# tlangin/MDQTPlasmaSims

Hardware: AMD Instinct MI355X
Metric: particle-steps/sec (MD+QT) at N=3.5k and N=1M; 1/2/4/8-GPU scaling (higher is better)
Workload: dtype f64

## Files before the change

mdqtplasmasims_amd/csrc/mdqt_engine.cpp:

```cpp
#include <errno.h>
#include <math.h>
#include <stdarg.h>
#include <stdio.h>
#include <stdlib.h>
#include <string.h>
#include <sys/stat.h>

#include <string>
#include <algorithm>
#include <memory>
#include <thread>
#include <vector>

#include <rccl/rccl.h>

#include "../../include/mdqt.h"
#include "mdqt_internal.hpp"
#include "mdqt_writer.hpp"
#include "mdqt_init_sample.hpp"

using namespace mdqt;

namespace {

// ... 124 lines not shown
    int fused_opt = 0;
    int last_fused = 0;
    int last_qt_kernel = 0;
    int last_qt_nseg = 0;
    int* dSpinErr = nullptr;
    unsigned long long* force_arrive = nullptr;
    hipStream_t sub_stream = nullptr;
    unsigned long long sub_target = 0;
    std::vector<int> spinUp;
    int nSpinUp = 0;
    int* dSpinUp = nullptr;
    double* dTkde = nullptr;
    int pumpBin0 = -2000;
    std::vector<double> vaHold;
    bool rs_pending = false;
    const double** dPeerParts = nullptr;
    int nslots = 0, npairs = 0, capPairs = 0;
    int2* dPairs = nullptr;
    int nsplit = 0;
    int nsplit_wg = 0;
    int split_opt = 1;
    int split_cus = 0;
    unsigned long long* dX48 = nullptr;
    int* dFlags = nullptr;
    bool guard = false;
    double* dU = nullptr;
    ncclComm_t comm = nullptr;
    double* dComm = nullptr;
    std::vector<mdqt_ctx*> local;
    size_t dCommCap = 0;
    double t = 0.;
    uint64_t qidx = 0;
    int c0 = 0;
    unsigned counter = 0;
    double Epot = 0., Epot0 = 0.;
    uint64_t x48 = 0;
    std::vector<double> Vholder;
    char saveDirectory[1024];
    std::unique_ptr<FileWriter> writer;
    FileWriter* shared_writer = nullptr;
    int init_threads = 0;
    bool timing = false;
    unsigned tkinds = 3;
    unsigned tperiod = 1, tcount[2] = {0, 0};
    unsigned toffset = 0;
    std::vector<hipEvent_t> evpool[4];
    int evused[4] = {0, 0, 0, 0};
    struct BdCall { hipEvent_t ag0 = nullptr, ag1 = nullptr; hipEvent_t m[7] = {}; };
    std::vector<BdCall> bdcalls;
    std::vector<hipEvent_t> bdfree;
    hipEvent_t bd_ag[2] = {nullptr, nullptr};
};

static int settle_forces(mdqt_ctx* s);
static int tail_check(mdqt_ctx* s);
static double u64_as_double(unsigned long long u) { double d; memcpy(&d, &u, sizeof d); return d; }

static int tail_reset(mdqt_ctx* s, bool keep_scale = false) {
    if (!keep_scale) s->tail_scale = 1.;
    s->tail_seen = 0;
    s->tail_pending = false;
    if (s->dTailSt) HIPCHK(hipMemsetAsync(s->dTailSt, 0, 16 * sizeof(unsigned long long), s->stream));
    return 0;
}

static int check_range_flag(mdqt_ctx* s) {
    if (s->dSpinErr) {
        int e = 0;
        if (hipMemcpyAsync(&e, s->dSpinErr, sizeof e, hipMemcpyDeviceToHost, s->stream) != hipSuccess ||
            hipStreamSynchronize(s->stream) != hipSuccess)
            return fail("reading the overlap flag failed");
        if (e) return fail("overlapped MD step: a QT launch timed out waiting for its force launch");
    }
    int f = 0;
    if (hipMemcpyAsync(&f, s->dFlags, sizeof f, hipMemcpyDeviceToHost, s->stream) != hipSuccess ||
        hipStreamSynchronize(s->stream) != hipSuccess)
        return fail("reading the position-range flag failed");
    if (f && !s->guard) {
        s->guard = true;
        return fail("positions left [-L/8, 9L/8] during the run (ion displacement > L/8 per half "
                    "substep); pair range checks are now on, but forces since the last sync used "
                    "the in-box minimum image");
    }
    return tail_check(s);
}


extern "C" void mdqt_default_params(mdqt_params* p) {
    memset(p, 0, sizeof(*p));
    p->Ge = 0.1; p->tmax = 30; p->density = 2; p->sig0 = 4.0; p->Te = 19.0; p->fracOfSig = 0;
    p->detuning = -1; p->detuningDP = 1; p->Om = 1; p->OmDP = 1;
    p->N0 = 3500; p->newRun = 1; p->c0 = 0; p->sampleFreq = 40; p->reNormalizewvFns = 0;
    p->qt_enabled = 1; p->rng_mode = 1; p->seed = 12345; p->job = 1;
    p->device = -1; p->world_size = 1; p->rank = 0; p->force_segments = 0; p->qt_model = 0;
    strcpy(p->saveDirectory, "dataLaserCool/");
    p->tpumpreal = 0.0000002; p->tstartV0 = 15;
}

extern "C" void mdqt_default_params_pump(mdqt_params* p, int qt_model) {
    mdqt_default_params(p);
    p->qt_model = qt_model;
    p->tmax = 25; p->Ge = 0.1; p->density = 2; p->N0 = 3500; p->sampleFreq = 40; p->tstartV0 = 15;
    if (qt_model == 2) {
        p->detuning = 0; p->Om = 2; p->tpumpreal = 0.0000001; strcpy(p->saveDirectory, "data/");
    } else if (qt_model == 3) {
        p->detuning = -1; p->Om = 1.3; p->tpumpreal = 0.0000001; strcpy(p->saveDirectory, "data422/");
    } else {
// ... 524 lines not shown
        return fail("the optical-pumping qt_models run on the Philox stream (rng_mode 1)");
    int ndev = 0;
    hipError_t e = hipGetDeviceCount(&ndev);
    if (e != hipSuccess || ndev < 1) return fail("no HIP device available (%s)", hipGetErrorString(e));
    mdqt_ctx* s = new mdqt_ctx();
    s->p = *p;
    s->p.saveDirectory[sizeof(s->p.saveDirectory) - 1] = 0;
    if (p->device >= 0) {
        if (p->device >= ndev) { delete s; return fail("device %d >= device count %d", p->device, ndev); }
        s->dev = p->device;
    } else {
        (void)hipGetDevice(&s->dev);
    }
    if (hipSetDevice(s->dev) != hipSuccess || hipStreamCreateWithFlags(&s->own, hipStreamNonBlocking) != hipSuccess) {
        delete s;
        return fail("cannot create HIP stream on device %d", p->device);
    }
    s->stream = s->own;
    if (hipMalloc(&s->dTab, sizeof(LaneTab)) != hipSuccess || hipMalloc(&s->dFTab, 2 * sizeof(FastTab)) != hipSuccess) {
        mdqt_destroy(s);
        return fail("hipMalloc lane tables");
    }
    {
        const int f[2] = {0, 1};
        if (hipMalloc(&s->dFlags, sizeof f) != hipSuccess ||
            hipMemcpy(s->dFlags, f, sizeof f, hipMemcpyHostToDevice) != hipSuccess) {
            mdqt_destroy(s);
            return fail("hipMalloc flags");
        }
    }
    build_constants(s);
    if (s->p.rng_mode == 0) {
        unsigned long long h[97];
        h[0] = srand48_state(s->p.seed);
        unsigned long long A = 0x5DEECE66Dull, Cc = 0xBull;
        for (int b = 0; b < 48; ++b) {
            h[1 + b] = A; h[49 + b] = Cc;
            Cc = (A * Cc + Cc) & 0xFFFFFFFFFFFFull;
            A = (A * A) & 0xFFFFFFFFFFFFull;
        }
        if (hipMalloc(&s->dX48, sizeof h) != hipSuccess ||
            hipMemcpy(s->dX48, h, sizeof h, hipMemcpyHostToDevice) != hipSuccess) {
            mdqt_destroy(s);
            return fail("drand48 state upload failed");
        }
    }
    if (hipMemcpy(s->dTab, &s->tab, sizeof(LaneTab), hipMemcpyHostToDevice) != hipSuccess ||
        hipMemcpy(s->dFTab, &s->ftab, sizeof(FastTab), hipMemcpyHostToDevice) != hipSuccess ||
        hipMemcpy(s->dFTab + 1, &s->ftabL, sizeof(FastTab), hipMemcpyHostToDevice) != hipSuccess) {
        mdqt_destroy(s);
        return fail("upload of the lane table failed");
    }
    s->t = 0.; s->qidx = 0; s->c0 = p->c0; s->counter = 0;
    s->x48 = srand48_state(p->seed);
    strncpy(s->saveDirectory, s->p.saveDirectory, sizeof(s->saveDirectory) - 1);
    s->saveDirectory[sizeof(s->saveDirectory) - 1] = 0;
    if (resize(s, 0)) { mdqt_destroy(s); return -1; }
    *out = s;
    return 0;
}

extern "C" void mdqt_destroy(mdqt_ctx* s) {
    if (!s) return;
    s->writer.reset();
    (void)hipSetDevice(s->dev);
    if (s->stream) (void)hipStreamSynchronize(s->stream);
    free_device(s);
    if (s->dTab) (void)hipFree(s->dTab);
    if (s->dFTab) (void)hipFree(s->dFTab);
    if (s->dComm) (void)hipFree(s->dComm);
    if (s->dSpinUp) (void)hipFree(s->dSpinUp);
    if (s->dArrive) (void)hipFree(s->dArrive);
    if (s->dSpinErr) (void)hipFree(s->dSpinErr);
    if (s->evQ) (void)hipEventDestroy(s->evQ);
    if (s->evS) (void)hipEventDestroy(s->evS);
    if (s->qs) (void)hipStreamDestroy(s->qs);
    if (s->dTkde) (void)hipFree(s->dTkde);
    if (s->dX48) (void)hipFree(s->dX48);
    if (s->dFlags) (void)hipFree(s->dFlags);
    if (s->comm) (void)ncclCommDestroy(s->comm);
    for (auto& pool : s->evpool)
        for (hipEvent_t ev : pool) (void)hipEventDestroy(ev);
    for (auto& c : s->bdcalls) {
        for (hipEvent_t ev : c.m) if (ev) (void)hipEventDestroy(ev);
        if (c.ag0) (void)hipEventDestroy(c.ag0);
        if (c.ag1) (void)hipEventDestroy(c.ag1);
    }
    for (hipEvent_t ev : s->bdfree) (void)hipEventDestroy(ev);
    for (hipEvent_t ev : s->bd_ag) if (ev) (void)hipEventDestroy(ev);
    if (s->own) (void)hipStreamDestroy(s->own);
    delete s;
}

static double tail_radius(int N, double L, double lDeb, int k, double* bound);
static double tail_radius_sum(const mdqt_ctx* s, double* bound);
static bool tail_measured(const mdqt_ctx* s);
static double skip_radius(const mdqt_ctx* s, double* bound);
static double far_radius(int N, double L, double lDeb, int k, double* bound);
static double far_radius_l(int N, double L, double lDeb, int k, int level, double* bound, bool cutterm = true);
static bool form_measured(const mdqt_ctx* s);
static double tier_radius(const mdqt_ctx* s, int k, int level, double* bound);
static void tier_radii(const mdqt_ctx* s, N3BArgs& a);
static double error_eps(const mdqt_ctx* s, const N3BArgs& a);
extern "C" double mdqt_get_const(const mdqt_ctx* s, const char* n) {
    if (!strcmp(n, "gamToEinsteinFreq")) return s->gamToE;
    if (!strcmp(n, "quantumTimestep")) return s->dtQ;
    if (!strcmp(n, "plasmaToQuantumTimestepRatio")) return s->ratio;
    if (!strcmp(n, "plasVelToQuantVel")) return s->pv2q;
    if (!strcmp(n, "vKick")) return s->vKick;
    if (!strcmp(n, "vKickDP")) return s->vKickDP;
    if (!strcmp(n, "lDeb")) return s->lDeb;
    if (!strcmp(n, "L")) return s->L;
    if (!strcmp(n, "decayRatioD5Halves")) return s->r;
    if (!strcmp(n, "kRat")) return s->kRat;
    if (!strcmp(n, "force_segments")) return s->nseg;
    if (!strcmp(n, "force_scheme")) return s->use_n3b ? 3 : s->use_n3 ? 2 : 1;
    if (!strcmp(n, "force_sort")) return s->use_n3b ? s->sort_mode : 0;
    if (!strcmp(n, "force_ax1")) return s->ax1_mode;
    if (!strcmp(n, "force_reduce_mask")) return s->tmask_mode;
    if (!strcmp(n, "force_tile_split")) return s->split_opt;
    if (!strcmp(n, "force_split_cus")) return s->split_cus;
    if (!strcmp(n, "force_tile_split_pairs")) return s->nsplit;
    if (!strcmp(n, "device_cus")) {
        int ncu = 0;
        return hipDeviceGetAttribute(&ncu, hipDeviceAttributeMultiprocessorCount, s->dev) == hipSuccess ? ncu : -1;
    }
    if (!strcmp(n, "force_balance")) return s->balance_opt;
    if (!strcmp(n, "force_balance_ratio")) return s->balance_ratio;
    if (!strcmp(n, "force_balance_ratio_equal")) return s->balance_ratio_eq;
    if (!strcmp(n, "n3b_block_lo")) return s->use_n3b ? s->n3b.Plo : 0;
    if (!strcmp(n, "n3b_block_hi")) return s->use_n3b ? s->n3b.Phi : 0;
    if (!strcmp(n, "force_skip_radius") || !strcmp(n, "force_tail_bound")) {
        double bound;
        const double r = (s->use_n3b && s->sort_mode == 1) ? skip_radius(s, &bound) : (bound = 0., s->L / 2.);
        if (n[6] == 's') return r;
// ... 82 lines not shown
    if (!strncmp(n, "gs", 2)) return s->gs[atoi(n + 2)];
    return NAN;
}


static int upload(mdqt_ctx* s, const double* R, const double* V, size_t ld, const double* psi,
                  const double* tPart) {
    const int N = s->N, S = s->S, W = s->p.world_size;
    HIPCHK(hipSetDevice(s->dev));
    if (R) {
        std::vector<double> h((size_t)3 * S * W, 0.);
        for (int g = 0; g < N; ++g) {
            const int w = g / S, l = g - w * S;
            for (int c = 0; c < 3; ++c) h[(size_t)w * 3 * S + (size_t)c * S + l] = R[(size_t)c * ld + g];
        }
        HIPCHK(hipMemcpyAsync(s->dR, h.data(), h.size() * sizeof(double), hipMemcpyHostToDevice, s->stream));
        int oor = 0;
        const double plo = -0.125 * s->L, phi = 1.125 * s->L;
        for (size_t k = 0; k < (size_t)3 * N && !oor; ++k) {
            const double x = R[(k / N) * ld + k % N];
            if (!(x >= plo && x <= phi)) oor = 1;
        }
        s->guard = oor != 0;
        const int zero = 0;
        HIPCHK(hipMemcpyAsync(s->dFlags, &zero, sizeof zero, hipMemcpyHostToDevice, s->stream));
        HIPCHK(hipStreamSynchronize(s->stream));
    }
    const int lo = s->lo, n = s->nloc;
    if (V) {
        std::vector<double> h((size_t)3 * S, 0.);
        for (int c = 0; c < 3; ++c)
            for (int i = 0; i < n; ++i) h[(size_t)c * S + i] = V[(size_t)c * ld + lo + i];
        HIPCHK(hipMemcpyAsync(s->dV, h.data(), h.size() * sizeof(double), hipMemcpyHostToDevice, s->stream));
        HIPCHK(hipStreamSynchronize(s->stream));
    }
    if (psi) {
        std::vector<double> h((size_t)24 * S, 0.);
        for (int i = 0; i < n; ++i)
            for (int k = 0; k < 24; ++k) h[(size_t)k * S + i] = psi[(size_t)(lo + i) * 24 + k];
        HIPCHK(hipMemcpyAsync(s->dPsi, h.data(), h.size() * sizeof(double), hipMemcpyHostToDevice, s->stream));
        HIPCHK(hipStreamSynchronize(s->stream));
    }
    if (tPart) {
        std::vector<double> h((size_t)S, 0.);
        for (int i = 0; i < n; ++i) h[i] = tPart[lo + i];
        HIPCHK(hipMemcpyAsync(s->dTp, h.data(), h.size() * sizeof(double), hipMemcpyHostToDevice, s->stream));
        HIPCHK(hipStreamSynchronize(s->stream));
    }
    return 0;
// ... 817 lines not shown
extern "C" int mdqt_step(mdqt_ctx* s) { return s ? run_substeps(s, 1, 1, 0, 0) : fail("NULL context"); }
extern "C" int mdqt_qstep(mdqt_ctx* s) { return s ? run_substeps(s, 1, 0, 1, 1) : fail("NULL context"); }
extern "C" int mdqt_substeps(mdqt_ctx* s, int n) {
    if (!s) return fail("NULL context");
    if (n < 0) return fail("negative substep count");
    return run_substeps(s, n, 1, 1, 1);
}

static bool overlap_applies(const mdqt_ctx* s) {
    return s->overlap_opt && s->p.world_size == 1 && s->local.empty() && s->use_n3 && s->nslots > 1 && s->qt_math == 2 &&
           s->p.qt_enabled && s->p.rng_mode == 1 && s->ratio <= MAXSUB && s->nloc > 0 &&
           (s->substep_mode == 2 || (s->substep_mode == 0 && s->nloc < kLaneKernelMaxIons));
}

static int arrive_setup(mdqt_ctx* s) {
    const int T = (s->N + 63) / 64;
    if (s->dArrive && s->arriveCap >= T) return 0;
    HIPCHK(hipStreamSynchronize(s->stream));
    if (s->qs) HIPCHK(hipStreamSynchronize(s->qs));
    if (s->dArrive) HIPCHK(hipFree(s->dArrive));
    s->dArrive = nullptr;
    HIPCHK(hipMalloc(&s->dArrive, (size_t)T * sizeof(unsigned long long)));
    HIPCHK(hipMemset(s->dArrive, 0, (size_t)T * sizeof(unsigned long long)));
    if (!s->dSpinErr) {
        HIPCHK(hipMalloc(&s->dSpinErr, sizeof(int)));
        HIPCHK(hipMemset(s->dSpinErr, 0, sizeof(int)));
    }
    HIPCHK(hipDeviceSynchronize());
    s->arriveCap = T;
    s->arriveEpoch = 0;
    return 0;
}

static int overlap_setup(mdqt_ctx* s) {
    if (arrive_setup(s)) return -1;
    if (s->qs) return 0;
    HIPCHK(hipStreamCreateWithFlags(&s->qs, hipStreamNonBlocking));
    HIPCHK(hipEventCreateWithFlags(&s->evQ, hipEventDisableTiming | hipEventDisableSystemFence));
    HIPCHK(hipEventCreateWithFlags(&s->evS, hipEventDisableTiming | hipEventDisableSystemFence));
    return 0;
}

static int md_steps_overlapped(mdqt_ctx* s, int n) {
    if (overlap_setup(s)) return -1;
    HIPCHK(hipEventRecord(s->evS, s->stream));
    HIPCHK(hipStreamWaitEvent(s->qs, s->evS, 0));
    for (int k = 0; k < n; ++k) {
        if (k > 0) HIPCHK(hipStreamWaitEvent(s->stream, s->evQ, 0));
        if (k > 0 && k % 64 == 0 && check_range_flag(s)) return -1;
        s->force_arrive = s->dArrive;
        const int rc = mdqt_forces(s);
        s->force_arrive = nullptr;
        if (rc) return -1;
        s->arriveEpoch += (unsigned long long)((s->N + 63) / 64);
        s->c0++;
        s->sub_stream = s->qs;
        s->sub_target = s->arriveEpoch;
        const int rq = run_substeps(s, s->ratio, 1, 1, 1);
        s->sub_stream = nullptr;
        if (rq) return -1;
        HIPCHK(hipEventRecord(s->evQ, s->qs));
    }
    HIPCHK(hipStreamWaitEvent(s->stream, s->evQ, 0));
    return 0;
}

static bool fused_applies(mdqt_ctx* s) {
    if (!(s->fused_opt && !s->overlap_opt && s->p.world_size == 1 && s->local.empty() && s->use_n3 && s->nslots > 1 &&
          s->qt_math == 2 && s->p.qt_enabled && s->p.rng_mode == 1 && s->ratio <= MAXSUB && s->nloc > 0 &&
          s->t > 0 && s->force_variant <= 1 &&
          (s->substep_mode == 2 || (s->substep_mode == 0 && s->nloc < kLaneKernelMaxIons))))
        return false;
// ... 14 lines not shown
    a.nseg = s->nslots;
    a.arrive = s->dArrive;
    a.arrive_target = s->arriveEpoch + T;
    a.spin_err = s->dSpinErr;
    a.arrive_sleep = 2;
    if (a.movmask != (m >= 32 ? 0xFFFFFFFFu : (1u << m) - 1u)) return fail("md_step_fused: t <= 0 in the interval");
    const bool tm = s->timing && (s->tkinds & 2u) && (s->tcount[1]++ % s->tperiod == s->toffset);
    hipEvent_t e0 = nullptr, e1 = nullptr;
    if (tm && take_events(s, 1, &e0, &e1)) return -1;
    HIPCHK(launch_md_step(f, a, s->dFTab, s->force_variant, s->stream, e0, e1));
    s->last_qt_kernel = QTK_MD_STEP;
    s->last_qt_nseg = a.nseg;
    s->arriveEpoch += T;
    s->f_pending = false;
    s->t = t;
    s->qidx += (uint64_t)m;
    return 0;
}

extern "C" int mdqt_md_steps(mdqt_ctx* s, int n) {
    if (!s) return fail("NULL context");
    if (n > 0 && overlap_applies(s)) return md_steps_overlapped(s, n);
    for (int k = 0; k < n; ++k) {
        if (k > 0 && k % 64 == 0 && check_range_flag(s)) return -1;
        if (fused_applies(s)) {
            if (local_reduce(s) || md_step_fused(s)) return -1;
            s->last_fused = 1;
            s->c0++;
            continue;
        }
        s->last_fused = 0;
        if (mdqt_allgather_positions(s)) return -1;
        if (mdqt_forces(s)) return -1;
        s->c0++;
        if (mdqt_substeps(s, s->ratio)) return -1;
    }
    return 0;
}

static int pairs_raw(int mode, int N, double L, double lDeb, const double* R, size_t ld, double* out,
                     int nseg_req, int device, int variant) {
    if (N < 1 || !R || !out || ld < (size_t)N) return fail("pairs_raw: bad arguments");
    if (variant < 0 || variant > 1) return fail("pairs_raw: variant must be 0 (exact) or 1 (fast)");
    int ndev = 0;
    if (hipGetDeviceCount(&ndev) != hipSuccess || ndev < 1) return fail("no HIP device available");
    if (device >= 0) HIPCHK(hipSetDevice(device));
    int lo, hi, S;
// ... 1169 lines not shown
```

mdqtplasmasims_amd/csrc/mdqt_ensemble.hpp:

```cpp
#pragma once

struct mdqt_ensemble {
    std::vector<mdqt_ctx*> jobs;
    int dev = 0;
    hipStream_t stream = nullptr;
    std::unique_ptr<FileWriter> writer;
    N3Args* dForce = nullptr;
    SubstepArgs* dSub = nullptr;
    int sub_blocks = 0;
    std::vector<N3Args> force_held;
    static constexpr int kRing = 8;
    char* ring = nullptr;
    size_t slot_bytes = 0;
    hipEvent_t ring_ev[kRing] = {};
    bool ring_used[kRing] = {};
    unsigned ring_pos = 0;
    int* hFlags = nullptr;
    int qt_waves = 0;
    bool timing = false;
    std::vector<hipEvent_t> evpool[2];
    int evused[2] = {0, 0};
};

namespace {

constexpr int kEnsembleMaxJobs = 1024;

int ens_job_params(const mdqt_params* base, int k, mdqt_params* out) {
    if (!base || !out) return fail("mdqt_ensemble_job_params: NULL argument");
    if (k < 0 || k >= kEnsembleMaxJobs) return fail("mdqt_ensemble_job_params: job index %d outside [0, %d)", k, kEnsembleMaxJobs);
    mdqt_params p = *base;
    p.job = base->job + (uint32_t)k;
    p.seed = base->seed + (uint32_t)k;
    *out = p;
    return 0;
}

int ens_ring_slot(mdqt_ensemble* e, char** slot, int* idx) {
    const int i = (int)(e->ring_pos++ % mdqt_ensemble::kRing);
    if (e->ring_used[i]) HIPCHK(hipEventSynchronize(e->ring_ev[i]));
// ... 108 lines not shown
        for (int k = 0; k < J; ++k) {
            mdqt_ctx* s = e->jobs[k];
            t = substep_args(s, h[k], m, 1, do_qt, 1);
            s->f_pending = false;
            maxn = std::max(maxn, h[k].n);
        }
        if (ens_upload(e, e->dSub, slot, (size_t)J * sizeof(SubstepArgs), idx)) return -1;
        hipEvent_t e0 = nullptr, e1 = nullptr;
        if (e->timing && ens_take_events(e, 1, &e0, &e1)) return -1;
        int inst = 0;
        HIPCHK(launch_substeps_r_ens(e->dSub, h[0], J, maxn, e->jobs[0]->dFTab, e->qt_waves, e->stream, e0, e1, &inst));
        for (int k = 0; k < J; ++k) {
            mdqt_ctx* s = e->jobs[k];
            s->last_qt_kernel = inst;
            s->last_qt_nseg = h[k].nseg;
            s->t = t;
            s->qidx += (uint64_t)m;
        }
        n -= m;
    }
    return 0;
}

int ens_range_flags(mdqt_ensemble* e) {
    const int J = (int)e->jobs.size();
    for (int k = 0; k < J; ++k)
        HIPCHK(hipMemcpyAsync(e->hFlags + k, e->jobs[k]->dFlags, sizeof(int), hipMemcpyDeviceToHost, e->stream));
    HIPCHK(hipStreamSynchronize(e->stream));
    int first = -1;
    for (int k = 0; k < J; ++k)
        if (e->hFlags[k] && !e->jobs[k]->guard) {
            e->jobs[k]->guard = true;
            if (first < 0) first = k;
        }
    if (first >= 0)
        return fail("job index %d: positions left [-L/8, 9L/8] during the run (ion displacement > L/8 per half "
                    "substep); pair range checks are now on, but forces since the last sync used the in-box "
                    "minimum image", first);
    return 0;
}

int ens_md_steps(mdqt_ensemble* e, int n) {
    const int J = (int)e->jobs.size();
    const int ratio = e->jobs[0]->ratio, per_step = (ratio + MAXSUB - 1) / MAXSUB;
    const int do_qt = e->jobs[0]->p.qt_enabled ? 1 : 0;
    bool tiles = true;
    for (const mdqt_ctx* s : e->jobs) tiles = tiles && s->use_n3;
    const int ahead = tiles ? std::min(64, e->sub_blocks / (J * per_step)) : 0;
    if (ahead < 2) {
        for (int k = 0; k < n; ++k) {
            if (k > 0 && k % 64 == 0 && ens_range_flags(e)) return -1;
            if (ens_forces(e)) return -1;
            for (mdqt_ctx* s : e->jobs) s->c0++;
            if (ens_substeps(e, ratio)) return -1;
        }
        return 0;
    }
    for (int k = 0; k < n;) {
        if (k > 0 && k % 64 == 0 && ens_range_flags(e)) return -1;
        const int b = std::min(std::min(n - k, ahead), 64 - k % 64);
        EnsForce f;
        if (ens_force_blocks(e, f)) return -1;
        char* slot = nullptr;
        int idx = 0;
        if (ens_ring_slot(e, &slot, &idx)) return -1;
        SubstepArgs* h = reinterpret_cast<SubstepArgs*>(slot);
        int nl = 0, maxn = 0;
        for (int st = 0; st < b; ++st) {
            for (int j = 0; j < J; ++j) {
                n3_forces_pending(e->jobs[j], f.h[j]);
                e->jobs[j]->c0++;
            }
            for (int rem = ratio; rem > 0; ++nl) {
                const int m = rem < MAXSUB ? rem : MAXSUB;
                for (int j = 0; j < J; ++j) {
                    mdqt_ctx* s = e->jobs[j];
                    SubstepArgs& a = h[(size_t)nl * J + j];
                    s->t = substep_args(s, a, m, 1, do_qt, 1);
                    s->qidx += (uint64_t)m;
                    s->f_pending = false;
                    maxn = std::max(maxn, a.n);
                }
// ... 18 lines not shown
        k += b;
    }
    return 0;
}

}

extern "C" int mdqt_ensemble_job_params(const mdqt_params* base, int k, mdqt_params* out) {
    return ens_job_params(base, k, out);
}

extern "C" void mdqt_ensemble_destroy(mdqt_ensemble* e) {
    if (!e) return;
    (void)hipSetDevice(e->dev);
    if (e->stream) (void)hipStreamSynchronize(e->stream);
    if (e->writer) (void)e->writer->flush(nullptr);
    for (size_t k = e->jobs.size(); k-- > 0;) {
        e->jobs[k]->shared_writer = nullptr;
        mdqt_destroy(e->jobs[k]);
    }
    if (e->dForce) (void)hipFree(e->dForce);
    if (e->dSub) (void)hipFree(e->dSub);
    if (e->ring) (void)hipHostFree(e->ring);
    if (e->hFlags) (void)hipHostFree(e->hFlags);
    for (hipEvent_t ev : e->ring_ev) if (ev) (void)hipEventDestroy(ev);
    for (auto& pool : e->evpool)
        for (hipEvent_t ev : pool) (void)hipEventDestroy(ev);
    delete e;
}

extern "C" int mdqt_ensemble_create(const mdqt_params* p, int njobs, mdqt_ensemble** out) {
    if (!p || !out) return fail("mdqt_ensemble_create: NULL argument");
    *out = nullptr;
    if (njobs < 1 || njobs > kEnsembleMaxJobs) return fail("mdqt_ensemble_create: njobs must be 1 .. %d", kEnsembleMaxJobs);
    if (p->world_size != 1) return fail("mdqt_ensemble_create: world_size must be 1 (an ensemble's jobs are whole systems on one device)");
    if (p->rng_mode != 1)
        return fail("mdqt_ensemble_create: rng_mode must be 1 (Philox): the drand48 order needs one substep per launch "
                    "and a resolve kernel per job");
    if (p->qt_model != 0) return fail("mdqt_ensemble_create: qt_model must be 0 (the SpeedUp program; the pump programs are not batched)");
    std::unique_ptr<mdqt_ensemble, void (*)(mdqt_ensemble*)> e(new (std::nothrow) mdqt_ensemble(), mdqt_ensemble_destroy);
    if (!e) return fail("mdqt_ensemble_create: out of memory");
    try {
        e->jobs.reserve((size_t)njobs);
        e->writer.reset(new FileWriter(std::min(16, 4 * njobs)));
    } catch (const std::exception& x) {
        return fail("mdqt_ensemble_create: %s", x.what());
    }
    for (int k = 0; k < njobs; ++k) {
        mdqt_params pk;
        mdqt_ctx* s = nullptr;
        if (ens_job_params(p, k, &pk) || mdqt_create(&pk, &s)) return -1;
        e->jobs.push_back(s);
        s->shared_writer = e->writer.get();
        if (k == 0) { e->dev = s->dev; e->stream = s->own; }
        if (s->qt_math != 2) return fail("mdqt_ensemble_create: qt_math must be 2");
        if (s->overlap_opt || s->fused_opt) return fail("mdqt_ensemble_create: the options overlap / fused_step are one system per launch");
        mdqt_set_stream(s, (void*)e->stream);
    }
    HIPCHK(hipSetDevice(e->dev));
    e->sub_blocks = std::max(njobs, 1024);
    e->slot_bytes = std::max((size_t)e->sub_blocks * sizeof(SubstepArgs), (size_t)njobs * sizeof(N3Args));
    if (hipMalloc(&e->dForce, (size_t)njobs * sizeof(N3Args)) != hipSuccess ||
        hipMalloc(&e->dSub, (size_t)e->sub_blocks * sizeof(SubstepArgs)) != hipSuccess ||
        hipHostMalloc((void**)&e->ring, e->slot_bytes * mdqt_ensemble::kRing, hipHostMallocDefault) != hipSuccess ||
        hipHostMalloc((void**)&e->hFlags, (size_t)njobs * sizeof(int), hipHostMallocDefault) != hipSuccess)
        return fail("mdqt_ensemble_create: allocating the argument blocks of %d jobs failed", njobs);
    for (hipEvent_t& ev : e->ring_ev) HIPCHK(hipEventCreateWithFlags(&ev, hipEventDisableTiming | hipEventDisableSystemFence));
    *out = e.release();
    return 0;
}

extern "C" int mdqt_ensemble_size(const mdqt_ensemble* e) { return e ? (int)e->jobs.size() : -1; }

extern "C" mdqt_ctx* mdqt_ensemble_job(mdqt_ensemble* e, int k) {
    if (!e || k < 0 || k >= (int)e->jobs.size()) {
        fail("mdqt_ensemble_job: job index %d outside the ensemble", k);
        return nullptr;
    }
    return e->jobs[(size_t)k];
}

extern "C" int mdqt_ensemble_set_option(mdqt_ensemble* e, const char* name, int value) {
    if (!e || !name) return fail("mdqt_ensemble_set_option: NULL argument");
    if (!strcmp(name, "qt_waves")) {
        if (value != 0 && value != 3) return fail("qt_waves must be 0 (the single-job kernel's register budget) or 3");
        e->qt_waves = value;
        return 0;
    }
// ... 38 lines not shown
    if (!e) return fail("NULL ensemble");
    for (mdqt_ctx* s : e->jobs)
        if (mdqt_setup_directories(s)) return -1;
    if (e->jobs[0]->p.newRun == 1) {
        if (mdqt_ensemble_init(e)) return -1;
    } else {
        for (mdqt_ctx* s : e->jobs) {
            s->c0 = s->p.c0;
            if (mdqt_read_conditions(s, s->c0)) return -1;
        }
    }
    if (ens_check(e, "mdqt_ensemble_run")) return -1;
    HIPCHK(hipSetDevice(e->dev));
    mdqt_ctx* a = e->jobs[0];
    const double tend = a->p.tmax + 0.0009;
    const int sf = a->p.sampleFreq, ratio = a->ratio;
    int tsc = ratio;
    long steps = 0;
    while (a->t <= tend) {
        if ((a->c0 + 1) % sf == 0 && tsc == 1)
            for (mdqt_ctx* s : e->jobs)
                if (output_async(s)) return -1;
        if (tsc == ratio) {
            if (steps > 0 && steps % 64 == 0 && ens_range_flags(e)) return -1;
            if (ens_forces(e)) return -1;
            for (mdqt_ctx* s : e->jobs) s->c0++;
            tsc = 0;
            steps++;
        }
        int n = 0, ts = tsc;
        double tt = a->t;
        do {
            n++; ts++; tt += a->dtQ;
        } while (n < MAXSUB && tt <= tend && !((a->c0 + 1) % sf == 0 && ts == 1) && ts != ratio);
        if (ens_substeps(e, n)) return -1;
        tsc += n;
    }
    for (mdqt_ctx* s : e->jobs)
        if (write_conditions_async(s, s->c0)) return -1;
    return flush_files(a);
}

extern "C" int mdqt_ensemble_enable_timing(mdqt_ensemble* e, int on) {
    if (!e) return fail("NULL ensemble");
    e->timing = on > 0;
    e->evused[0] = e->evused[1] = 0;
    return 0;
// ... 25 lines not shown
```

mdqtplasmasims_amd/csrc/mdqt_qtfast.hip:

```cpp
#include "mdqt_device.hpp"
#include "mdqt_pairs.hpp"

#include <math.h>

#include <type_traits>

namespace mdqt {

#ifndef MDQT_LANE_WG
#define MDQT_LANE_WG 256
#endif
constexpr int kLaneWG = MDQT_LANE_WG;
static_assert(kLaneWG % 64 == 0 && kLaneWG <= 256, "lane kernel workgroup: whole waves, <= 256 threads");
static_assert(!MDQT_QT_SCTAB || kLaneWG >= 128, "the sincos table is staged by the first 128 threads");
#ifndef MDQT_EXPT_ROWS
#define MDQT_EXPT_ROWS 4
#endif
constexpr int kRows = MDQT_EXPT_ROWS;
static_assert(kRows == 1 || kRows == 2 || kRows == 4, "ions per wave");
constexpr int kLaneIons = kLaneWG / 64 * kRows;

__device__ __forceinline__ double rsq_nr(double x) { return rsq3(x); }
__device__ __forceinline__ double nrm2(cxd y) { return fma(y.re, y.re, y.im * y.im); }
__device__ __forceinline__ double rho_im_r(cxd a, cxd b) { return fma(a.im, b.re, -(a.re * b.im)); }
// ... 292 lines not shown
}

#if defined(MDQT_EXPT_QTSTAMPS)
__device__ unsigned long long g_qt_stamps[16 * 4096];
#define QT_STAMP(slot, v) (st_[slot] = (v))
#define QT_JCOUNT(c) (st_[7] += (__builtin_amdgcn_ballot_w64(c) != 0))
#else
#define QT_STAMP(slot, v) ((void)0)
#define QT_JCOUNT(c) ((void)0)
#endif

#if defined(MDQT_EXPT_MDSTAMPS)
__device__ unsigned long long g_md_stamps[4 * 4096];
#endif

#ifndef MDQT_LANE_WPE
#define MDQT_LANE_WPE 0
#endif
#if MDQT_LANE_WPE > 0
#define LANE_WPE_ATTR __attribute__((amdgpu_waves_per_eu(MDQT_LANE_WPE, MDQT_LANE_WPE)))
#else
#define LANE_WPE_ATTR
#endif
template <bool DPPX, bool FAST, bool FUSED, bool IM01 = false, bool EDZ = false, bool NORN = false>
__device__ __forceinline__ void lane_substeps(const SubstepArgs& a, const FastTab* __restrict__ tab, int blk) {
#if defined(MDQT_EXPT_QTSTAMPS)
    unsigned long long st_[16] = {};
#endif
    QT_STAMP(0, __builtin_amdgcn_s_memtime());
    QT_STAMP(4, __builtin_amdgcn_s_memrealtime());
    const int k = threadIdx.x & 15;
    const int grp = threadIdx.x >> 4;
    const int iraw = kRows == 4 ? blk * (kLaneWG / 16) + grp
                                : (blk * (kLaneWG / 64) + (grp >> 2)) * kRows + ((grp & 3) % kRows);
    const bool store = iraw < a.n && (kRows == 4 || (grp & 3) < kRows);
    const int i = store ? iraw : a.n - 1;
    const QTConst& qc = a.qc;
    const int S = a.S;
    const int st = DPPX ? state_of_lane0(k) : k;
    const int cy = DPPX ? 9 : 12, cz = DPPX ? 10 : 13;
    const int c = (k == cy) ? 1 : (k == cz) ? 2 : 0;
    const bool owner = (k == 0) || (k == cy) || (k == cz);
    const int base = threadIdx.x & ~15;
    const int l0 = base + tab->col[0][k], l1 = base + tab->col[1][k], l2 = base + tab->col[2][k];
    const cxd c0 = {tab->cre[0][k], tab->cim[0][k]}, c1 = {tab->cre[1][k], tab->cim[1][k]};
    const double c2re = tab->cre[2][k], c2im = tab->cim[2][k], dms = tab->dms[k], dmc = tab->dmc[k];
    const double mre = tab->mre[k], mi0 = tab->mi0[k], mi1 = tab->mi1[k], hdp = tab->hdp[k];
// ... 143 lines not shown
        pp = half_drift(pp, vv, f, moving, DT, DT2, L);
        vv = vv + dt * f;
        pp = half_drift(pp, vv, f, moving, DT, DT2, L);
    };
    QT_STAMP(1, __builtin_amdgcn_s_memtime());
    if (!FAST && !a.do_qt) {
        if (a.do_step)
            for (int s = 0; s < a.nsub; ++s) drift(p, v, s);
    } else {
        if (FAST || a.do_step) drift(p, v, 0);
        double pre_p = p, pre_v = v;
        double sn, cs;
        double u = EDZ ? v * pv2q_v : v * pv2q_v + edt[0];
        double tn = tPart + dtq_v;
        sincos_q2((u * cphi) * tn, sct, sn, cs);
#if defined(MDQT_EXPT_PHASEROT)
        double phi_c = (u * cphi) * tn;
#endif
#ifndef MDQT_QT_UNROLL
#define MDQT_QT_UNROLL 2
#endif
#ifndef MDQT_PHASE_BOUND
#define MDQT_PHASE_BOUND 1
#endif
        bool phase_small = false;
        if constexpr (FAST && EDZ && DPPX && MDQT_PHASE_BOUND) {
            const double vb = fabs(v) + (double)(a.nsub + 1) * (fabs(dt * f) + qc.kickmax);
            const double tb = fabs(tPart) + (double)(a.nsub + 1) * dtq_v;
            const double pb = ((vb * fabs(pv2q_v)) * fabs(cphi)) * tb;
            phase_small = __builtin_amdgcn_ballot_w64(!(pb < 524288.)) == 0;
        }
        auto substep = [&](int s, auto chk) {
            tPart = tn;
            const double dp = DPPX ? lane_sum_p8(nrm2(w) * hdp, one) : lane_sum_p(nrm2(w) * hdp);
            const double u1 = su[grp][s][0], u2 = su[grp][s][1];
            cxd w0, w1, w2;
            exchange(w, w0, w1, w2);
            double kick;
#if defined(MDQT_EXPT_NOJUMP)
            const bool nojump = true;
            (void)u1;
#else
            const bool nojump = u1 > dp;
#endif
            QT_JCOUNT(!nojump);
            double vn, pn, un, phin, snn, csn;
// ... 12 lines not shown
                    const bool adv = a.do_step && s + 1 < a.nsub;
                    pn = adv ? pd : pn;
                    vn = adv ? vd : vn;
                }
                un = EDZ ? vn * pv2q_v : vn * pv2q_v + edt[s1];
                tn = tPart + dtq_v;
                phin = (un * cphi) * tn;
#if defined(MDQT_EXPT_PHASEROT)
                {
                    const double dph = phin - phi_c, z = dph * dph;
                    const double sd = dph * fma(z, fma(z, fma(z, -1.984126984126984e-04, 8.333333333333333e-03),
                                                       -1.666666666666667e-01), 1.0);
                    const double cd = fma(z, fma(z, fma(z, fma(z, 2.48015873015873e-05, -1.388888888888889e-03),
                                                        4.166666666666666e-02), -0.5), 1.0);
                    snn = fma(sn, cd, cs * sd);
                    csn = fma(cs, cd, -(sn * sd));
                    phi_c = phin;
                }
#else
                if (MDQT_QT_SCTAB) sincos_tab(phin, sct, snn, csn);
                else sincos_fast(phin, snn, csn);
#endif
            };
            if (nojump) {
                {
                    const double kt = kick_term(w, w0, w1, w2, kw0, kw1, kw2);
                    kick = DPPX ? lane_sum_p8(kt, one) : lane_sum_p(kt);
                }
                next_phase();
                const cxd md = {mre, fma(mi1, u, mi0)};
                const cxd c2 = {fma(dms, sn, c2re), fma(dmc, cs, c2im)};
                cxd y = w, acc = {0., 0.};
                cxd y0 = w0, y1 = w1, y2 = w2;
#pragma unroll
                for (int stg = 0; stg < 4; ++stg) {
                    double dpy = dp;
                    if (stg > 0) {
                        dpy = DPPX ? lane_sum_p8(nrm2(y) * hdp, one) : lane_sum_p(nrm2(y) * hdp);
                        exchange(y, y0, y1, y2);
                    }
                    const double pref = rsq_nr(1. - dpy);
                    const cxd ws = IM01 ? row_r_im01(md, y, c0.im, y0, c1.im, y1, c2, y2)
                                        : row_r(md, y, c0, y0, c1, y1, c2, y2);
                    const cxd d = {fma(pref, ws.re, -y.re), fma(pref, ws.im, -y.im)};
                    if (stg == 0) acc = d;
                    else if (stg < 3) acc = {fma(3., d.re, acc.re), fma(3., d.im, acc.im)};
                    else acc = {acc.re + d.re, acc.im + d.im};
                    if (stg < 2) y = {fma(0.5, d.re, w.re), fma(0.5, d.im, w.im)};
                    else if (stg == 2) y = {w.re + d.re, w.im + d.im};
                }
                w = {fma(0.125, acc.re, w.re), fma(0.125, acc.im, w.im)};
            } else {
                tPart = 0;
                const double nk = sq(w);
                double n3, n4, n5, n6;
                if constexpr (DPPX) {
                    n3 = dpp<BCAST(0)>(nk); n4 = dpp<BCAST(4)>(nk); n5 = dpp<BCAST(3)>(nk); n6 = dpp<BCAST(7)>(nk);
                } else {
                    n3 = dpp<BCAST(2)>(nk); n4 = dpp<BCAST(3)>(nk); n5 = dpp<BCAST(4)>(nk); n6 = dpp<BCAST(5)>(nk);
                }
                double randDOrS, randDir, rand3, dummy;
                if (a.U) {
                    draw_pair(qc, a.U, S, i, gid, a.q0 + (uint64_t)s, 1, randDOrS, randDir);
                    draw_pair(qc, a.U, S, i, gid, a.q0 + (uint64_t)s, 2, rand3, dummy);
                    (void)dummy;
                } else {
                    double x0, x1;
                    philox_pair(qc, gid, a.q0 + (uint64_t)s, k < 8 ? 1 : 2, x0, x1);
                    randDOrS = dpp<BCAST(0)>(x0);
                    randDir = dpp<BCAST(0)>(x1);
                    rand3 = dpp<BCAST(8)>(x0);
                }
                const int target = (DPPX || qc.model == 0)
                                       ? jump_target(qc, n3, n4, n5, n6, u2, randDOrS, randDir, rand3, kick)
                                       : jump_target_pump(qc, n3, n4, n5, n6, u2, randDOrS, randDir, rand3, kick);
                w = {st == target ? 1. : 0., 0.};
                next_phase();
            }
            if constexpr (decltype(chk)::value)
                if (!(fabs(phin) < 1048576.)) sincos(phin, &snn, &csn);
            if (!NORN && qc.renorm) w = [&] {
                const double r = rsq_nr(lane_norm16(nrm2(w), one));
                return cxd{w.re * r, w.im * r};
            }();
            v = vn;
            p = pn;
            u = un;
            sn = snn;
            cs = csn;
        };
        auto loop = [&](auto chk) {
            if (MDQT_QT_UNROLL == 2) {
                int s = 0;
                for (; s + 1 < a.nsub; s += 2) {
                    substep(s, chk);
                    substep(s + 1, chk);
                }
                if (s < a.nsub) substep(s, chk);
// ... 177 lines not shown
        if (rnd < nr[0]) up = 1;
        else if (rnd < nr[0] + nr[2]) up = r2 < 1. / 3;
        else if (rnd < nr[0] + nr[2] + nr[3]) up = r2 < 2. / 3;
        else up = 0;
    } else {
        if (rnd < nr[0] + nr[2]) up = 1;
        else if (rnd < nr[0] + nr[2] + nr[3]) up = r2 < 2. / 3;
        else if (rnd < nr[0] + nr[2] + nr[3] + nr[4]) up = r2 < 1. / 3;
        else up = 0;
    }
    tags[i] = up;
}

hipError_t launch_tag_spin_up(const double* psi, int n, int S, uint64_t gid0, uint64_t q, const QTConst& qc,
                              int* tags, hipStream_t s) {
    if (n <= 0) return hipSuccess;
    hipLaunchKernelGGL(k_tag_spin_up, dim3((n + 255) / 256), dim3(256), 0, s, psi, n, S, gid0, q, qc, tags);
    return hipGetLastError();
}

#endif

#if defined(MDQT_ENSEMBLE_TU)
#define LANE_ENS_KERNELS(SUFFIX, ATTR)                                                                              \
    template <bool DPPX, bool FAST>                                                                                 \
    __global__ __launch_bounds__(256) ATTR void k_substeps_lanes_r_ens##SUFFIX(const SubstepArgs* __restrict__ jobs, \
                                                                               const FastTab* __restrict__ tab) {   \
        const SubstepArgs& a = jobs[blockIdx.y];                                                                    \
        if ((int)blockIdx.x * kLaneIons >= a.n) return;                                                             \
        lane_substeps<DPPX, FAST, false>(a, tab, blockIdx.x);                                                       \
    }                                                                                                               \
    template <bool DPPX, bool EDZ, bool NORN = false>                                                               \
    __global__ __launch_bounds__(256) ATTR void k_substeps_lanes_im_ens##SUFFIX(const SubstepArgs* __restrict__ jobs, \
                                                                                const FastTab* __restrict__ tab) {  \
        const SubstepArgs& a = jobs[blockIdx.y];                                                                    \
        if ((int)blockIdx.x * kLaneIons >= a.n) return;                                                             \
        lane_substeps<DPPX, true, false, true, EDZ, NORN>(a, tab, blockIdx.x);                                      \
    }
LANE_ENS_KERNELS(, LANE_WPE_ATTR)
LANE_ENS_KERNELS(_w3, __attribute__((amdgpu_waves_per_eu(3, 3))))
#undef LANE_ENS_KERNELS

#ifndef MDQT_IM01
#define MDQT_IM01 1
#endif
#ifndef MDQT_EDZ
#define MDQT_EDZ 1
#endif
#ifndef MDQT_NORN
#define MDQT_NORN 1
#endif
hipError_t launch_substeps_r_ens(const SubstepArgs* jobs, const SubstepArgs& a, int njobs, int max_n, const FastTab* tab,
                                 int wpe, hipStream_t s, hipEvent_t ev0, hipEvent_t ev1, int* instance) {
    if (njobs <= 0 || max_n <= 0 || a.nsub <= 0) return hipSuccess;
    if (!jobs || njobs > 65535 || a.nsub > MAXSUB || a.qc.model != 0 || a.arrive || a.U) return hipErrorInvalidValue;
    if (wpe != 0 && wpe != 3) return hipErrorInvalidValue;
    const dim3 gl((max_n + kLaneIons - 1) / kLaneIons, njobs), bl(kLaneWG);
    const FastTab* lt = tab + 1;
    const uint64_t all = (1ull << a.nsub) - 1;
    const bool allmove = a.do_step && a.do_qt && a.nseg >= 1 && (a.movmask & all) == all;
    int inst;
#define LANE_ENS_LAUNCH(KERNEL, ...)                                                                    \
    do {                                                                                                \
// ... 30 lines not shown
```

Baseline: 2.812 billion.

## Poll range flags via mapped host memory and make QT jump path wave-uniform

Moves the position-range and overlap-error flags into coherent mapped host memory, so the host can poll them every step without a device-to-host copy and a stream synchronize. The ensemble per-job flag copies are dropped as well, with a full drain only where a check must be definitive. Separately, the QT substep kernel now takes a fast RK-only path when a wave ballot shows no lane jumps. Otherwise every lane runs both the RK and jump computations and selects results, which avoids divergent branches at the cost of redundant work in mixed waves. Polling without a sync can read a flag late, and device writes to host-coherent memory may be slower.

```diff
diff --git a/mdqtplasmasims_amd/csrc/mdqt_engine.cpp b/mdqtplasmasims_amd/csrc/mdqt_engine.cpp
--- a/mdqtplasmasims_amd/csrc/mdqt_engine.cpp
+++ b/mdqtplasmasims_amd/csrc/mdqt_engine.cpp
@@ -170,6 +170,7 @@
     int split_opt = 1;
     int split_cus = 0;
     unsigned long long* dX48 = nullptr;
+    volatile int* hFlags = nullptr;
     int* dFlags = nullptr;
     bool guard = false;
     double* dU = nullptr;
@@ -212,25 +213,24 @@
     return 0;
 }
 
-static int check_range_flag(mdqt_ctx* s) {
-    if (s->dSpinErr) {
-        int e = 0;
-        if (hipMemcpyAsync(&e, s->dSpinErr, sizeof e, hipMemcpyDeviceToHost, s->stream) != hipSuccess ||
-            hipStreamSynchronize(s->stream) != hipSuccess)
-            return fail("reading the overlap flag failed");
-        if (e) return fail("overlapped MD step: a QT launch timed out waiting for its force launch");
-    }
-    int f = 0;
-    if (hipMemcpyAsync(&f, s->dFlags, sizeof f, hipMemcpyDeviceToHost, s->stream) != hipSuccess ||
-        hipStreamSynchronize(s->stream) != hipSuccess)
-        return fail("reading the position-range flag failed");
-    if (f && !s->guard) {
+static int poll_flags(mdqt_ctx* s) {
+    if (s->hFlags[1]) return fail("overlapped MD step: a QT launch timed out waiting for its force launch");
+    if (s->hFlags[0] && !s->guard) {
         s->guard = true;
         return fail("positions left [-L/8, 9L/8] during the run (ion displacement > L/8 per half "
                     "substep); pair range checks are now on, but forces since the last sync used "
                     "the in-box minimum image");
     }
+    return 0;
+}
+static int check_range_flag(mdqt_ctx* s) {
+    if (hipStreamSynchronize(s->stream) != hipSuccess) return fail("reading the position-range flag failed");
+    if (poll_flags(s)) return -1;
     return tail_check(s);
+}
+static int loop_check(mdqt_ctx* s, int k) {
+    if (poll_flags(s)) return -1;
+    return (k > 0 && k % 64 == 0) ? tail_check(s) : 0;
 }
 
 
@@ -801,12 +801,19 @@
         return fail("hipMalloc lane tables");
     }
     {
-        const int f[2] = {0, 1};
-        if (hipMalloc(&s->dFlags, sizeof f) != hipSuccess ||
-            hipMemcpy(s->dFlags, f, sizeof f, hipMemcpyHostToDevice) != hipSuccess) {
+        void *h = nullptr, *d = nullptr;
+        if (hipHostMalloc(&h, 2 * sizeof(int), hipHostMallocMapped | hipHostMallocCoherent | hipHostMallocPortable) != hipSuccess) {
             mdqt_destroy(s);
-            return fail("hipMalloc flags");
-        }
+            return fail("hipHostMalloc flags");
+        }
+        s->hFlags = (volatile int*)h;
+        s->hFlags[0] = s->hFlags[1] = 0;
+        if (hipHostGetDevicePointer(&d, h, 0) != hipSuccess) {
+            mdqt_destroy(s);
+            return fail("hipHostGetDevicePointer flags");
+        }
+        s->dFlags = (int*)d;
+        s->dSpinErr = s->dFlags + 1;
     }
     build_constants(s);
     if (s->p.rng_mode == 0) {
@@ -850,13 +857,12 @@
     if (s->dComm) (void)hipFree(s->dComm);
     if (s->dSpinUp) (void)hipFree(s->dSpinUp);
     if (s->dArrive) (void)hipFree(s->dArrive);
-    if (s->dSpinErr) (void)hipFree(s->dSpinErr);
     if (s->evQ) (void)hipEventDestroy(s->evQ);
     if (s->evS) (void)hipEventDestroy(s->evS);
     if (s->qs) (void)hipStreamDestroy(s->qs);
     if (s->dTkde) (void)hipFree(s->dTkde);
     if (s->dX48) (void)hipFree(s->dX48);
-    if (s->dFlags) (void)hipFree(s->dFlags);
+    if (s->hFlags) (void)hipHostFree((void*)s->hFlags);
     if (s->comm) (void)ncclCommDestroy(s->comm);
     for (auto& pool : s->evpool)
         for (hipEvent_t ev : pool) (void)hipEventDestroy(ev);
@@ -890,6 +896,7 @@
     if (!strcmp(n, "vKickDP")) return s->vKickDP;
     if (!strcmp(n, "lDeb")) return s->lDeb;
     if (!strcmp(n, "L")) return s->L;
+    if (!strcmp(n, "range_guard")) return s->guard ? 1 : 0;
     if (!strcmp(n, "decayRatioD5Halves")) return s->r;
     if (!strcmp(n, "kRat")) return s->kRat;
     if (!strcmp(n, "force_segments")) return s->nseg;
@@ -1018,9 +1025,8 @@
             if (!(x >= plo && x <= phi)) oor = 1;
         }
         s->guard = oor != 0;
-        const int zero = 0;
-        HIPCHK(hipMemcpyAsync(s->dFlags, &zero, sizeof zero, hipMemcpyHostToDevice, s->stream));
         HIPCHK(hipStreamSynchronize(s->stream));
+        s->hFlags[0] = 0;
     }
     const int lo = s->lo, n = s->nloc;
     if (V) {
@@ -1884,10 +1890,6 @@
     s->dArrive = nullptr;
     HIPCHK(hipMalloc(&s->dArrive, (size_t)T * sizeof(unsigned long long)));
     HIPCHK(hipMemset(s->dArrive, 0, (size_t)T * sizeof(unsigned long long)));
-    if (!s->dSpinErr) {
-        HIPCHK(hipMalloc(&s->dSpinErr, sizeof(int)));
-        HIPCHK(hipMemset(s->dSpinErr, 0, sizeof(int)));
-    }
     HIPCHK(hipDeviceSynchronize());
     s->arriveCap = T;
     s->arriveEpoch = 0;
@@ -1909,7 +1911,7 @@
     HIPCHK(hipStreamWaitEvent(s->qs, s->evS, 0));
     for (int k = 0; k < n; ++k) {
         if (k > 0) HIPCHK(hipStreamWaitEvent(s->stream, s->evQ, 0));
-        if (k > 0 && k % 64 == 0 && check_range_flag(s)) return -1;
+        if (loop_check(s, k)) return -1;
         s->force_arrive = s->dArrive;
         const int rc = mdqt_forces(s);
         s->force_arrive = nullptr;
@@ -1970,7 +1972,7 @@
     if (!s) return fail("NULL context");
     if (n > 0 && overlap_applies(s)) return md_steps_overlapped(s, n);
     for (int k = 0; k < n; ++k) {
-        if (k > 0 && k % 64 == 0 && check_range_flag(s)) return -1;
+        if (loop_check(s, k)) return -1;
         if (fused_applies(s)) {
             if (local_reduce(s) || md_step_fused(s)) return -1;
             s->last_fused = 1;
diff --git a/mdqtplasmasims_amd/csrc/mdqt_ensemble.hpp b/mdqtplasmasims_amd/csrc/mdqt_ensemble.hpp
--- a/mdqtplasmasims_amd/csrc/mdqt_ensemble.hpp
+++ b/mdqtplasmasims_amd/csrc/mdqt_ensemble.hpp
@@ -15,7 +15,6 @@
     hipEvent_t ring_ev[kRing] = {};
     bool ring_used[kRing] = {};
     unsigned ring_pos = 0;
-    int* hFlags = nullptr;
     int qt_waves = 0;
     bool timing = false;
     std::vector<hipEvent_t> evpool[2];
@@ -170,14 +169,12 @@
     return 0;
 }
 
-int ens_range_flags(mdqt_ensemble* e) {
+int ens_range_flags(mdqt_ensemble* e, bool drain = true) {
     const int J = (int)e->jobs.size();
-    for (int k = 0; k < J; ++k)
-        HIPCHK(hipMemcpyAsync(e->hFlags + k, e->jobs[k]->dFlags, sizeof(int), hipMemcpyDeviceToHost, e->stream));
-    HIPCHK(hipStreamSynchronize(e->stream));
+    if (drain) HIPCHK(hipStreamSynchronize(e->stream));
     int first = -1;
     for (int k = 0; k < J; ++k)
-        if (e->hFlags[k] && !e->jobs[k]->guard) {
+        if (e->jobs[k]->hFlags[0] && !e->jobs[k]->guard) {
             e->jobs[k]->guard = true;
             if (first < 0) first = k;
         }
@@ -197,7 +194,7 @@
     const int ahead = tiles ? std::min(64, e->sub_blocks / (J * per_step)) : 0;
     if (ahead < 2) {
         for (int k = 0; k < n; ++k) {
-            if (k > 0 && k % 64 == 0 && ens_range_flags(e)) return -1;
+            if (ens_range_flags(e, false)) return -1;
             if (ens_forces(e)) return -1;
             for (mdqt_ctx* s : e->jobs) s->c0++;
             if (ens_substeps(e, ratio)) return -1;
@@ -205,7 +202,7 @@
         return 0;
     }
     for (int k = 0; k < n;) {
-        if (k > 0 && k % 64 == 0 && ens_range_flags(e)) return -1;
+        if (ens_range_flags(e, false)) return -1;
         const int b = std::min(std::min(n - k, ahead), 64 - k % 64);
         EnsForce f;
         if (ens_force_blocks(e, f)) return -1;
@@ -270,7 +267,6 @@
     if (e->dForce) (void)hipFree(e->dForce);
     if (e->dSub) (void)hipFree(e->dSub);
     if (e->ring) (void)hipHostFree(e->ring);
-    if (e->hFlags) (void)hipHostFree(e->hFlags);
     for (hipEvent_t ev : e->ring_ev) if (ev) (void)hipEventDestroy(ev);
     for (auto& pool : e->evpool)
         for (hipEvent_t ev : pool) (void)hipEventDestroy(ev);
@@ -310,8 +306,7 @@
     e->slot_bytes = std::max((size_t)e->sub_blocks * sizeof(SubstepArgs), (size_t)njobs * sizeof(N3Args));
     if (hipMalloc(&e->dForce, (size_t)njobs * sizeof(N3Args)) != hipSuccess ||
         hipMalloc(&e->dSub, (size_t)e->sub_blocks * sizeof(SubstepArgs)) != hipSuccess ||
-        hipHostMalloc((void**)&e->ring, e->slot_bytes * mdqt_ensemble::kRing, hipHostMallocDefault) != hipSuccess ||
-        hipHostMalloc((void**)&e->hFlags, (size_t)njobs * sizeof(int), hipHostMallocDefault) != hipSuccess)
+        hipHostMalloc((void**)&e->ring, e->slot_bytes * mdqt_ensemble::kRing, hipHostMallocDefault) != hipSuccess)
         return fail("mdqt_ensemble_create: allocating the argument blocks of %d jobs failed", njobs);
     for (hipEvent_t& ev : e->ring_ev) HIPCHK(hipEventCreateWithFlags(&ev, hipEventDisableTiming | hipEventDisableSystemFence));
     *out = e.release();
@@ -396,7 +391,7 @@
             for (mdqt_ctx* s : e->jobs)
                 if (output_async(s)) return -1;
         if (tsc == ratio) {
-            if (steps > 0 && steps % 64 == 0 && ens_range_flags(e)) return -1;
+            if (ens_range_flags(e, false)) return -1;
             if (ens_forces(e)) return -1;
             for (mdqt_ctx* s : e->jobs) s->c0++;
             tsc = 0;
diff --git a/mdqtplasmasims_amd/csrc/mdqt_qtfast.hip b/mdqtplasmasims_amd/csrc/mdqt_qtfast.hip
--- a/mdqtplasmasims_amd/csrc/mdqt_qtfast.hip
+++ b/mdqtplasmasims_amd/csrc/mdqt_qtfast.hip
@@ -338,7 +338,7 @@
 #else
 #define LANE_WPE_ATTR
 #endif
-template <bool DPPX, bool FAST, bool FUSED, bool IM01 = false, bool EDZ = false, bool NORN = false>
+template <bool DPPX, bool FAST, bool FUSED, bool IM01 = false, bool EDZ = false, bool NORN = false, bool JUNI = !FUSED>
 __device__ __forceinline__ void lane_substeps(const SubstepArgs& a, const FastTab* __restrict__ tab, int blk) {
 #if defined(MDQT_EXPT_QTSTAMPS)
     unsigned long long st_[16] = {};
@@ -528,6 +528,9 @@
 #endif
 #ifndef MDQT_PHASE_BOUND
 #define MDQT_PHASE_BOUND 1
+#endif
+#ifndef MDQT_JUMP_UNIFORM
+#define MDQT_JUMP_UNIFORM 1
 #endif
         bool phase_small = false;
         if constexpr (FAST && EDZ && DPPX && MDQT_PHASE_BOUND) {
@@ -586,12 +589,11 @@
                 else sincos_fast(phin, snn, csn);
 #endif
             };
-            if (nojump) {
-                {
-                    const double kt = kick_term(w, w0, w1, w2, kw0, kw1, kw2);
-                    kick = DPPX ? lane_sum_p8(kt, one) : lane_sum_p(kt);
-                }
-                next_phase();
+            auto rk_kick = [&]() {
+                const double kt = kick_term(w, w0, w1, w2, kw0, kw1, kw2);
+                return DPPX ? lane_sum_p8(kt, one) : lane_sum_p(kt);
+            };
+            auto rk_stages = [&]() {
                 const cxd md = {mre, fma(mi1, u, mi0)};
                 const cxd c2 = {fma(dms, sn, c2re), fma(dmc, cs, c2im)};
                 cxd y = w, acc = {0., 0.};
@@ -613,9 +615,9 @@
                     if (stg < 2) y = {fma(0.5, d.re, w.re), fma(0.5, d.im, w.im)};
                     else if (stg == 2) y = {w.re + d.re, w.im + d.im};
                 }
-                w = {fma(0.125, acc.re, w.re), fma(0.125, acc.im, w.im)};
-            } else {
-                tPart = 0;
+                return cxd{fma(0.125, acc.re, w.re), fma(0.125, acc.im, w.im)};
+            };
+            auto jump = [&](auto tape, double& jkick) {
                 const double nk = sq(w);
                 double n3, n4, n5, n6;
                 if constexpr (DPPX) {
@@ -624,7 +626,7 @@
                     n3 = dpp<BCAST(2)>(nk); n4 = dpp<BCAST(3)>(nk); n5 = dpp<BCAST(4)>(nk); n6 = dpp<BCAST(5)>(nk);
                 }
                 double randDOrS, randDir, rand3, dummy;
-                if (a.U) {
+                if constexpr (decltype(tape)::value) {
                     draw_pair(qc, a.U, S, i, gid, a.q0 + (uint64_t)s, 1, randDOrS, randDir);
                     draw_pair(qc, a.U, S, i, gid, a.q0 + (uint64_t)s, 2, rand3, dummy);
                     (void)dummy;
@@ -635,9 +637,39 @@
                     randDir = dpp<BCAST(0)>(x1);
                     rand3 = dpp<BCAST(8)>(x0);
                 }
-                const int target = (DPPX || qc.model == 0)
-                                       ? jump_target(qc, n3, n4, n5, n6, u2, randDOrS, randDir, rand3, kick)
-                                       : jump_target_pump(qc, n3, n4, n5, n6, u2, randDOrS, randDir, rand3, kick);
+                return (DPPX || qc.model == 0)
+                           ? jump_target(qc, n3, n4, n5, n6, u2, randDOrS, randDir, rand3, jkick)
+                           : jump_target_pump(qc, n3, n4, n5, n6, u2, randDOrS, randDir, rand3, jkick);
+            };
+            if constexpr (JUNI && MDQT_JUMP_UNIFORM) {
+            auto jump_substep = [&](auto tape) {
+                const double kick_rk = rk_kick();
+                const cxd w_rk = rk_stages();
+                double kick_j;
+                const int target = jump(tape, kick_j);
+                w = {nojump ? w_rk.re : (st == target ? 1. : 0.), nojump ? w_rk.im : 0.};
+                kick = nojump ? kick_rk : kick_j;
+                tPart = nojump ? tPart : 0.;
+                next_phase();
+            };
+            if (__builtin_expect(__builtin_amdgcn_ballot_w64(!nojump) == 0, 1)) {
+                kick = rk_kick();
+                next_phase();
+                w = rk_stages();
+            } else if (a.U) {
+                jump_substep(std::true_type{});
+            } else {
+                jump_substep(std::false_type{});
+            }
+            } else if (nojump) {
+                kick = rk_kick();
+                next_phase();
+                w = rk_stages();
+            } else {
+                tPart = 0;
+                int target;
+                if (a.U) target = jump(std::true_type{}, kick);
+                else target = jump(std::false_type{}, kick);
                 w = {st == target ? 1. : 0., 0.};
                 next_phase();
             }
@@ -861,23 +893,23 @@
 #endif
 
 #if defined(MDQT_ENSEMBLE_TU)
-#define LANE_ENS_KERNELS(SUFFIX, ATTR)                                                                              \
+#define LANE_ENS_KERNELS(SUFFIX, ATTR, JUNI)                                                                        \
     template <bool DPPX, bool FAST>                                                                                 \
     __global__ __launch_bounds__(256) ATTR void k_substeps_lanes_r_ens##SUFFIX(const SubstepArgs* __restrict__ jobs, \
                                                                                const FastTab* __restrict__ tab) {   \
         const SubstepArgs& a = jobs[blockIdx.y];                                                                    \
         if ((int)blockIdx.x * kLaneIons >= a.n) return;                                                             \
-        lane_substeps<DPPX, FAST, false>(a, tab, blockIdx.x);                                                       \
+        lane_substeps<DPPX, FAST, false, false, false, false, JUNI>(a, tab, blockIdx.x);                            \
     }                                                                                                               \
     template <bool DPPX, bool EDZ, bool NORN = false>                                                               \
     __global__ __launch_bounds__(256) ATTR void k_substeps_lanes_im_ens##SUFFIX(const SubstepArgs* __restrict__ jobs, \
                                                                                 const FastTab* __restrict__ tab) {  \
         const SubstepArgs& a = jobs[blockIdx.y];                                                                    \
         if ((int)blockIdx.x * kLaneIons >= a.n) return;                                                             \
-        lane_substeps<DPPX, true, false, true, EDZ, NORN>(a, tab, blockIdx.x);                                      \
-    }
-LANE_ENS_KERNELS(, LANE_WPE_ATTR)
-LANE_ENS_KERNELS(_w3, __attribute__((amdgpu_waves_per_eu(3, 3))))
+        lane_substeps<DPPX, true, false, true, EDZ, NORN, JUNI>(a, tab, blockIdx.x);                                \
+    }
+LANE_ENS_KERNELS(, LANE_WPE_ATTR, true)
+LANE_ENS_KERNELS(_w3, __attribute__((amdgpu_waves_per_eu(3, 3))), false)
 #undef LANE_ENS_KERNELS
 
 #ifndef MDQT_IM01
```

New measurement: 2.885 billion (median of 6 runs). 2.6% higher.
